# pinellolab/crispr-bean

Measured on AMD Instinct MI355X. Metric: SVI steps/sec, 50k-guide x 20-sample sorting model, higher is better.
Workload: dtype f64; 1 GPU; variant sorting MixtureNormal: 50000 guides x 5 reps x (4 sort bins + bulk), 10000 targets; one SVI step = draw + ELBO + grad + ClippedAdam; per GPU; config=metric, guides=50000, guides_this_rank=50000, n_reps=5, n_condits=5, parallelism=one screen per GPU x1, loss all-reduce every 100 steps, graph_chunk=64

## Files before the change

crispr-bean_amd/csrc/bean_async_v2.hpp:

```cpp
#pragma once

#include "bean_devargs_sgpr.hpp"

#ifndef BEAN_ASYNC_INLINE
#define BEAN_ASYNC_INLINE __forceinline__
#endif
#ifndef BEAN_ASYNC_PRIO
#define BEAN_ASYNC_PRIO 1
#endif
#ifndef BEAN_ASYNC_SLEEP
#define BEAN_ASYNC_SLEEP 8
#endif
#ifndef BEAN_ASYNC_EU
#define BEAN_ASYNC_EU BEAN_WAVE_EU
#endif

namespace bean {

constexpr long kAsyncMinItems = 2800;
constexpr long kAsyncMaxItems = 24000;
__host__ __device__ inline int async_waves_per_simd(long items, long simds = 1024) {
    const double per_simd = (double)items / (double)(simds > 0 ? simds : 1);
    return per_simd <= 5400.0 / 1024.0 ? 2 : (per_simd <= 11000.0 / 1024.0 ? 3 : 4);
}
__host__ __device__ inline bool async_size_in_range(long items, long simds = 1024) {
    const double per_simd = (double)items / (double)(simds > 0 ? simds : 1);
    return per_simd >= (double)kAsyncMinItems / 1024.0 && per_simd <= (double)kAsyncMaxItems / 1024.0;
}
__host__ __device__ inline bool async_finisher_roles(int waves_per_simd, long items, long simds) {
    const double per_wave = (double)items / (double)(waves_per_simd * simds);
    return (waves_per_simd == 2 && per_wave >= 0.95) || (waves_per_simd == 3 && per_wave >= 2.4);
}
constexpr int kAsyncQueueStride = 32;
constexpr int kAsyncStealEvery = 64;
constexpr int kAsyncSpinMax = 1 << 21;

struct AsyncArgs {
    unsigned long long step0, slot0;
    int n_steps;
    int* queue;
    int* done;
    int* abort_flag;
    int n_guide_blocks;
    int fin_split;
    int* fhead;
    int* fring;
    long fring_stride;
    const float* step_sizes;
    unsigned long long* stamps;
};
constexpr int kAsyncStampStep0 = 40, kAsyncStampSteps = 4;
constexpr long kAsyncStampFinOff = 1l << 22;
#ifdef BEAN_ASYNC_STAMP
#define BEAN_ASYNC_T(k)                                                                              \
    if (st_row) {                                                                                    \
        unsigned long long u_;                                                                       \
        asm volatile("s_memrealtime %0\n\ts_waitcnt lgkmcnt(0)" : "=s"(u_)::"memory");               \
        if (lane == 0) st_row[k] = u_;                                                               \
    }
#define BEAN_ASYNC_TF(k)                                                                             \
    if (st_row) {                                                                                    \
        unsigned long long u_;                                                                       \
        asm volatile("s_memrealtime %0\n\ts_waitcnt lgkmcnt(0)" : "=s"(u_)::"memory");               \
        if (lane == 0) st_row[kAsyncStampFinOff + (k)] = u_;                                         \
    }
#define BEAN_ASYNC_ST_ARG , unsigned long long* st_row
#define BEAN_ASYNC_ST_PASS , st_row
#define BEAN_ASYNC_ST_DRAW , (st_row ? st_row + 3 : nullptr)
#else
#define BEAN_ASYNC_T(k)
#define BEAN_ASYNC_TF(k)
#define BEAN_ASYNC_ST_ARG
#define BEAN_ASYNC_ST_PASS
#define BEAN_ASYNC_ST_DRAW
#endif

__global__ __launch_bounds__(64) void k_put_args(DevArgs c, DevArgs* out) {
    const unsigned int* src = (const unsigned int*)&c;
    unsigned int* dst = (unsigned int*)out;
    for (unsigned i = threadIdx.x; i < sizeof(DevArgs) / 4; i += 64) dst[i] = src[i];
}

__global__ __launch_bounds__(256) void k_step_sizes(DevArgs c, unsigned long long step0, int n, float* out) {
    const int i = blockIdx.x * blockDim.x + threadIdx.x;
    if (i < n) out[i] = adam_coef(c, step0 + (unsigned long long)i + 1).step_size;
}

__global__ __launch_bounds__(256) void k_async_head(DevArgs c, AsyncArgs a, DevArgs* args_out, int* ws, int ws_ints,
                                                    float* step_sizes) {
    const long tid = (long)blockIdx.x * 256 + threadIdx.x, nth = (long)gridDim.x * 256;
    for (long i = tid; i < 8 * a.fring_stride; i += nth) a.fring[i] = 0;
    if (blockIdx.x != 0) return;
    for (int i = threadIdx.x; i < ws_ints; i += 256) ws[i] = 0;
    for (int i = threadIdx.x; i < c.n_arrival_ctr; i += 256) c.tile_ctr[i] = 0;
    for (int i = threadIdx.x; i < a.n_steps; i += 256) step_sizes[i] = adam_coef(c, a.step0 + (unsigned long long)i + 1).step_size;
    const unsigned int* src = (const unsigned int*)&c;
    unsigned int* dst = (unsigned int*)args_out;
    for (unsigned i = threadIdx.x; i < sizeof(DevArgs) / 4; i += 256) dst[i] = src[i];
    if (threadIdx.x != 0) return;
    StepCtr last, next;
    last.step = a.step0 + a.n_steps - 1;
    last.slot = a.slot0 + a.n_steps - 1;
    last.step_size = adam_coef(c, last.step + 1).step_size;
    last.pad_ = 0.f;
    next.step = last.step + 1;
    next.slot = last.slot + 1;
    next.step_size = 0.f;
    next.pad_ = 0.f;
    *c.ctrA = last;
    *c.ctrB = next;
}

__device__ __forceinline__ void async_give_up(const DevArgs* cp, const AsyncArgs& a) {
    __hip_atomic_store(a.abort_flag, 1, __ATOMIC_RELAXED, __HIP_MEMORY_SCOPE_AGENT);
    long long* acc = cp->loss_acc;
    for (int i = 0; i < a.n_steps; ++i)
        atomicAdd((unsigned long long*)(acc + ((long)(a.slot0 + i) * kLossSub) * kLossWords) + 2, 1ull);
}

constexpr int kAsyncFinDone = 0, kAsyncFinLeave = 1, kAsyncFinGaveUp = 2;
template <int FAM, bool ACC>
__device__ BEAN_ASYNC_INLINE int async_finish_tile(const DevArgs* cp, unsigned long long step, unsigned long long slot,
                                              float step_size, int tile, int part, const int* wait_slot,
                                              const int* abort_flag BEAN_ASYNC_ST_ARG) {
    if (BEAN_ASYNC_PRIO && !wait_slot) __builtin_amdgcn_s_setprio(3);
    const DevArgs c = dev_args_in_sgprs(cp);
    part = rfl_i(part);
    step = rfl_u64(step);
    slot = rfl_u64(slot);
    step_size = __builtin_bit_cast(float, rfl_i(__builtin_bit_cast(int, step_size)));
    tile = rfl_i(tile);
    int t0, nt;
    {
        const int gf = tile * 64 - c.g_sh > 0 ? tile * 64 - c.g_sh : 0;
        const int gl = tile * 64 + 63 - c.g_sh < c.G ? tile * 64 + 63 - c.g_sh : c.G - 1;
        const int gv = c.g2t[threadIdx.x == 0 ? gf : gl];
        t0 = __builtin_amdgcn_readlane(gv, 0);
        nt = __builtin_amdgcn_readlane(gv, 1) - t0 + 1;
    }
    StepCtr ctr;
    ctr.step = step;
    ctr.slot = slot;
    ctr.step_size = step_size;
    ctr.pad_ = 0.f;
    constexpr bool MIX = FAM == kMixture;
    constexpr int COH = 2;
    extern __shared__ double tabs[];
    const int lane = threadIdx.x, R = c.R, G = c.G, B = c.B;
    const int t1 = t0 + nt - 1;
    int tof0, tof1;
    {
        const int tv = c.toff[lane == 0 ? t0 : t1 + 1];
        tof0 = __builtin_amdgcn_readlane(tv, 0);
        tof1 = __builtin_amdgcn_readlane(tv, 1);
    }
    if (wait_slot) {
        int spins = 0;
        for (;;) {
            int v = 0, ab = 0;
            if (lane == 0) v = __hip_atomic_load(wait_slot, __ATOMIC_RELAXED, __HIP_MEMORY_SCOPE_AGENT);
            if (lane == 1) ab = __hip_atomic_load(abort_flag, __ATOMIC_RELAXED, __HIP_MEMORY_SCOPE_AGENT);
            if (__any(ab != 0)) return kAsyncFinLeave;
            if (__builtin_amdgcn_readfirstlane(v) != 0) break;
            if (++spins > kAsyncSpinMax) return kAsyncFinGaveUp;
            __builtin_amdgcn_s_sleep(BEAN_ASYNC_SLEEP);
        }
        if (BEAN_ASYNC_PRIO) __builtin_amdgcn_s_setprio(3);
    }
    asm volatile("" ::: "memory");
    BEAN_ASYNC_TF(part == 2 ? 6 : 4);
    const unsigned long long s_prep = ctr.step + 1;
    AdamCoef ak;
    ak.step_size = ctr.step_size;
    ak.clip = (float)c.clip;
    const int g_first = tile * 64 - c.g_sh > 0 ? tile * 64 - c.g_sh : 0;
    const int g_last = tile * 64 + 63 - c.g_sh < G ? tile * 64 + 63 - c.g_sh : G - 1;
    const bool left_str = tof0 < g_first;
    const bool right_str = tof1 > g_last + 1;
    long long loss_hi = 0, loss_lo = 0, loss_bad = 0;
    auto loss_term = [&](double v) {
        if (!(fabs(v) < kLossPartMax)) {
            loss_bad = 1;
            return;
        }
        const double hi = rint(v * 1024.0);
        loss_hi += (long long)hi;
        loss_lo += (long long)rint((v - hi * (1.0 / 1024.0)) * 1099511627776.0);
    };
    if (part & 1) {
    int own_left = left_str ? 0 : 1, own_right = right_str ? 0 : 1;
    {
        int* const bp = c.bnd_ctr + (lane == 0 ? (left_str ? tile - 1 : tile) : tile);
        int old = 0;
        if ((lane == 0 && left_str) || (lane == 1 && right_str))
            old = __hip_atomic_fetch_add(bp, 1, __ATOMIC_RELAXED, __HIP_MEMORY_SCOPE_AGENT);
        const int ol = __builtin_amdgcn_readlane(old, 0), orr = __builtin_amdgcn_readlane(old, 1);
        if (left_str && (ol & 1)) own_left = 1;
        if (right_str && (orr & 1)) own_right = 1;
    }
    BEAN_ASYNC_TF(0);
    const int ta = own_left ? t0 : t0 + 1, tb = own_right ? t1 : t1 - 1;
    double* hmu = tabs;
    double* hy = tabs + 64;
    __syncthreads();

    {
        const int j = lane & 3;
        float* const P = j == 0 ? c.p[0] : (j == 1 ? c.p[1] : (j == 2 ? c.p[2] : c.p[3]));
        float* const M = j == 0 ? c.m[0] : (j == 1 ? c.m[1] : (j == 2 ? c.m[2] : c.m[3]));
        float* const V = j == 0 ? c.v[0] : (j == 1 ? c.v[1] : (j == 2 ? c.v[2] : c.v[3]));
        for (int base = ta; base <= tb; base += 16) {
            const int t = base + (lane >> 2);
            const bool act = t <= tb;
            const int tc = act ? t : tb;
            int2 dsc;
            dsc.x = 0;
            dsc.y = 2;
            if (!c.tsum_direct) dsc = c.tdesc[tc];
            const int n = dsc.y * R, ntm = c.tile_targets;
            const long S = c.tsum_direct ? 2 * (long)c.T : (long)c.n_tiles * ntm;
            float pj = coh_ld<COH>(P + tc), mj = coh_ld<COH>(M + tc), vj = coh_ld<COH>(V + tc);
            const float p1 = coh_ld<COH>(c.p[1] + tc), p3 = coh_ld<COH>(c.p[3] + tc);
            const double eps1 = coh_ld<COH>(c.eps_mu + tc), eps2 = coh_ld<COH>(c.eps_sd + tc);
            const double mu = coh_ld<COH>(c.mu_t + tc), y = coh_ld<COH>(c.y_t + tc);
            double am[4] = {0.0, 0.0, 0.0, 0.0}, ay[4] = {0.0, 0.0, 0.0, 0.0};
            const float rR = 1.0f / (float)R;
            for (int i0 = 0; i0 < n; i0 += 32) {
                double xm[2][4], xy[2][4];
#pragma unroll
                for (int mm = 0; mm < 2; ++mm)
#pragma unroll
                    for (int k = 0; k < 4; ++k) {
                        const int i = i0 + 16 * mm + j + 4 * k;
                        xm[mm][k] = 0.0;
                        xy[mm][k] = 0.0;
                        if (act && i < n) {
                            const int part = (int)(((float)i + 0.5f) * rR), rr = i - part * R;
                            const long o = (long)rr * S + (c.tsum_direct ? 2 * (long)tc + part
                                                                         : (part == 0 ? dsc.x : (dsc.x / ntm + part) * ntm));
                            xm[mm][k] = row_ld<true>(c.tsum + o);
                            xy[mm][k] = row_ld<true>(c.tsum + (long)R * S + o);
                        }
                    }
#pragma unroll
                for (int mm = 0; mm < 2; ++mm)
#pragma unroll
                    for (int k = 0; k < 4; ++k) {
                        const int i = i0 + 16 * mm + j + 4 * k;
                        if (act && i < n) {
                            am[k] += xm[mm][k];
                            ay[k] += xy[mm][k];
                        }
                    }
            }
            double gmu = (am[0] + am[2]) + (am[1] + am[3]);
            double gy = (ay[0] + ay[2]) + (ay[1] + ay[3]);
            gmu += __shfl_xor(gmu, 2, 64);
            gy += __shfl_xor(gy, 2, 64);
            gmu += __shfl_xor(gmu, 1, 64);
            gy += __shfl_xor(gy, 1, 64);
            double dlogp_mu, dlogp_dy, lt;
            tgt_prior_terms(c, tc, tgt_sd_prior(c, tc), mu, y, eps1, eps2, p1, p3, dlogp_mu, dlogp_dy, lt);
            if (act && j == 0) loss_term(lt);
            const double Gd = j < 2 ? gmu - dlogp_mu : gy - dlogp_dy;
            const double grad = tgt_grad(j, Gd, j < 2 ? eps1 : eps2, exp((double)pj));
            adam_update(pj, mj, vj, (float)grad, ak);
            if (act) {
                coh_st<COH>(P + t, pj);
                coh_st<COH>(M + t, mj);
                coh_st<COH>(V + t, vj);
            }
            const float2 nrm = normal2_at(c.seed, ((unsigned long long)kSiteTarget << 48) + (unsigned long long)(c.t_off + tc),
                                          s_prep * 4ull);
            const double en = j < 2 ? (double)nrm.x : (double)nrm.y;
            const float p_scale = __shfl_xor(pj, 1, 64);
            const double val = tgt_draw(pj, en, p_scale);
            if (act && (j & 1) == 0) {
                coh_st<COH>((j == 0 ? c.eps_mu : c.eps_sd) + t, en);
                coh_st<COH>((j == 0 ? c.mu_t : c.y_t) + t, val);
                (j == 0 ? hmu : hy)[t - ta] = val;
            }
        }
    }
    __syncthreads();
    BEAN_ASYNC_TF(1);
    {
#pragma clang fp contract(off)
        const int nue = c.ue_idx[2 * B];
        const int nu1 = nue > 0 ? nue : 1, per = 64 / nu1;
        double* const ecdf = tabs + 128;
        double* const epdf = ecdf + 64;
        double* const eupd = epdf + 64;
        for (int base = ta; base <= tb; base += per) {
            const int grp = lane / nu1, ue = lane - grp * nu1;
            const int t = base + grp;
            const bool live = grp < per && t <= tb && nue > 0;
            const int tl = live ? t - ta : 0;
            {
                const double mu = hmu[tl], y = hy[tl];
                const double sigma = c.family == kNormal ? exp(0.5 * y) : exp(y);
                const double inv = 1.0 / sigma;
                const double u = (c.ue_z[live ? ue : 0] - mu) * inv;
                const double pdf = norm_pdf(u);
                if (live) {
                    ecdf[lane] = norm_cdf(u);
                    epdf[lane] = pdf;
                    eupd[lane] = u * pdf;
                }
            }
            __syncthreads();
            const int cnt = (tb - base + 1 < per ? tb - base + 1 : per) * B;
            for (int q = lane; q < cnt; q += 64) {
                const int gq = q / B, b = q - gq * B, tq = base + gq;
                const double y = hy[tq - ta];
                const double sigma = c.family == kNormal ? exp(0.5 * y) : exp(y);
                const double dsig_dy = c.family == kNormal ? 0.5 * sigma : sigma;
                const double inv = 1.0 / sigma;
                const int ih = c.ue_idx[b], il = c.ue_idx[B + b];
                const double ch = ih < 0 ? 1.0 : ecdf[gq * nu1 + ih], cl = il < 0 ? 0.0 : ecdf[gq * nu1 + il];
                const double fh = ih < 0 ? 0.0 : epdf[gq * nu1 + ih], fl = il < 0 ? 0.0 : epdf[gq * nu1 + il];
                const double uh = ih < 0 ? 0.0 : eupd[gq * nu1 + ih], ul = il < 0 ? 0.0 : eupd[gq * nu1 + il];
                const long o = (long)b * c.T + tq;
                coh_st<COH>(c.tabP + o, ch - cl);
                coh_st<COH>(c.tabPmu + o, -(fh - fl) * inv);
                coh_st<COH>(c.tabPy + o, -(uh - ul) * inv * dsig_dy);
            }
            __syncthreads();
        }
    }
    }
    BEAN_ASYNC_TF(2);
    if (MIX && (part & 2)) {
        const int g = tile * 64 + lane - c.g_sh;
        double lg = 0.0;
        if (g >= 0 && g < G) {
            param_guide_mix<true, true, true, COH>(c, g, ak, s_prep, lg);
            loss_term(lg);
        }
    }
    BEAN_ASYNC_TF(3);
    if (part & 1) {
        for (int r0 = 0; r0 < R; r0 += 64) {
            if (r0 + lane < R) {
                const long long* o = c.lpart + 3 * (long)(((tile >> 3) * R + r0 + lane) * 8 + (tile & 7));
                loss_hi += __hip_atomic_load(o, __ATOMIC_RELAXED, __HIP_MEMORY_SCOPE_AGENT);
                loss_lo += __hip_atomic_load(o + 1, __ATOMIC_RELAXED, __HIP_MEMORY_SCOPE_AGENT);
                loss_bad += __hip_atomic_load(o + 2, __ATOMIC_RELAXED, __HIP_MEMORY_SCOPE_AGENT);
            }
        }
    }
    loss_hi = wave_sum_i64(loss_hi);
    loss_lo = wave_sum_i64(loss_lo);
    loss_bad = wave_sum_i64(loss_bad);
    if (lane == 0) {
        long long a = 0, b = 0, d = 0;
        a += loss_hi;
        b += loss_lo;
        d += loss_bad;
        long long* acc = c.loss_acc + ((long)ctr.slot * kLossSub + (tile & (kLossSub - 1))) * kLossWords;
        atomicAdd((unsigned long long*)acc, (unsigned long long)a);
        atomicAdd((unsigned long long*)acc + 1, (unsigned long long)b);
        if (d) atomicAdd((unsigned long long*)acc + 2, (unsigned long long)d);
    }
    return kAsyncFinDone;
}

template <int FAM, bool ACC>
__device__ BEAN_ASYNC_INLINE int2 async_guide_item(const DevArgs& c, W2Prep& pp, bool stage_now, unsigned long long step,
                                              unsigned long long slot, float step_size, int tile,
                                              int r BEAN_ASYNC_ST_ARG) {
    StepCtr ctr;
    ctr.step = rfl_u64(step);
    ctr.slot = rfl_u64(slot);
    ctr.step_size = __builtin_bit_cast(float, rfl_i(__builtin_bit_cast(int, step_size)));
    ctr.pad_ = 0.f;
    const int lane = threadIdx.x, R = c.R;
    const int wg = ((tile >> 3) * R + r) * 8 + (tile & 7);
    int t0, nt;
    double tot;
    guide_wave2_rest<FAM, ACC, 2>(c, ctr, tile, r, wg, pp, stage_now, t0, nt, tot BEAN_ASYNC_ST_DRAW);
    BEAN_ASYNC_T(4);
    if (lane == 0) {
        long long w0 = 0, w1 = 0, w2 = 1;
        if (fabs(tot) < kLossPartMax) {
            const double hi = rint(tot * 1024.0);
            w0 = (long long)hi;
            w1 = (long long)rint((tot - hi * (1.0 / 1024.0)) * 1099511627776.0);
            w2 = 0;
        }
        long long* o = c.lpart + 3 * (long)wg;
        __hip_atomic_store(o, w0, __ATOMIC_RELAXED, __HIP_MEMORY_SCOPE_AGENT);
        __hip_atomic_store(o + 1, w1, __ATOMIC_RELAXED, __HIP_MEMORY_SCOPE_AGENT);
        __hip_atomic_store(o + 2, w2, __ATOMIC_RELAXED, __HIP_MEMORY_SCOPE_AGENT);
    }
    asm volatile("s_waitcnt vmcnt(0)" ::: "memory");
    int last = 0;
    if (lane == 0) {
        const int old = __hip_atomic_fetch_add(c.tile_ctr + tile, 1, __ATOMIC_RELAXED, __HIP_MEMORY_SCOPE_AGENT);
        if (old % R == R - 1) last = 1;
    }
    last = __builtin_amdgcn_readfirstlane(last);
// ... 77 lines not shown
            int w = __hip_atomic_load(pw, __ATOMIC_RELAXED, __HIP_MEMORY_SCOPE_AGENT);
            asm volatile("" ::: "memory");
            const DevArgs c = dev_args_in_sgprs(cp);
            const int tile_u = rfl_i(tile), r_u = rfl_i(r);
            const unsigned long long step = a.step0 + (unsigned long long)s, slot = a.slot0 + (unsigned long long)s;
            W2Prep pp;
            guide_wave2_prepare<FAM, ACC, 2>(c, rfl_u64(step), tile_u, r_u, pp);
            int v = need ? w : s, ab = lane == 4 ? w : 0;
            if (__any(ab != 0)) return;
            bool ready = __all(v >= s);
            const bool fast = ready;
            if (!ready) {
                {
                    const int lane_st = w2_lane_here();
                    guide_wave2_stage_counts<FAM>(c, lane_st, tile_u, r_u, pp);
                    guide_wave2_stage<FAM, 3>(c, lane_st, tile_u, r_u, pp);
                }
                int spins = 0;
                for (;;) {
                    if (++spins > kAsyncSpinMax) {
                        if (lane == 0) async_give_up(cp, a);
                        return;
                    }
                    if (roles && (spins & (kAsyncStealEvery - 1)) == 0) {
                        int e = 0;
                        if (lane == 0) {
                            const int h = __hip_atomic_load(fhead, __ATOMIC_RELAXED, __HIP_MEMORY_SCOPE_AGENT);
                            if (h < total_fin) {
                                const int cand = __hip_atomic_load(fring + h, __ATOMIC_RELAXED, __HIP_MEMORY_SCOPE_AGENT);
                                int expect = h;
                                if (cand != 0 && __hip_atomic_compare_exchange_strong(fhead, &expect, h + 1, __ATOMIC_RELAXED,
                                                                                      __ATOMIC_RELAXED, __HIP_MEMORY_SCOPE_AGENT))
                                    e = h + 1;
                            }
                        }
                        e = __builtin_amdgcn_readfirstlane(e);
                        if (e != 0) {
                            int jt;
                            async_fin_pos(e - 1, nx, a.fin_split, fin_s, jt, fin_part);
                            fin_tile = jt * 8 + x;
                            break;
                        }
                    }
                    __builtin_amdgcn_s_sleep(BEAN_ASYNC_SLEEP);
                    w = __hip_atomic_load(pw, __ATOMIC_RELAXED, __HIP_MEMORY_SCOPE_AGENT);
                    v = need ? w : s;
                    ab = lane == 4 ? w : 0;
                    if (__any(ab != 0)) return;
                    if (__all(v >= s)) {
                        ready = true;
                        break;
                    }
                }
            }
            asm volatile("" ::: "memory");
            BEAN_ASYNC_T(1);
            if (ready) {
                const int2 fin = async_guide_item<FAM, ACC>(c, pp, fast, step, slot, a.step_sizes[s], tile_u, r_u BEAN_ASYNC_ST_PASS);
                item = -1;
                BEAN_ASYNC_T(2);
                if (fin.x >= 0) {
                    if (roles) {
                        if (lane == 0) {
                            int* const w = fring + (long)(s * nx + jt) * (a.fin_split ? 2 : 1);
                            __hip_atomic_store(w, s + 1, __ATOMIC_RELAXED, __HIP_MEMORY_SCOPE_AGENT);
                            if (a.fin_split) __hip_atomic_store(w + 1, s + 1, __ATOMIC_RELAXED, __HIP_MEMORY_SCOPE_AGENT);
                        }
                    } else {
                        fin_s = s;
                        fin_tile = tile;
                        fin_part = 3;
                    }
                }
            }
        }
        if (fin_s >= 0) {
#ifdef BEAN_ASYNC_STAMP
            st_row = nullptr;
            if (a.stamps && fin_s >= kAsyncStampStep0 && fin_s < kAsyncStampStep0 + kAsyncStampSteps)
                st_row = a.stamps + ((long)(fin_s - kAsyncStampStep0) * ((long)((n_tiles + 7) / 8 * 8) * R) + (long)fin_tile * R) * 8;
#endif
            const unsigned long long step = a.step0 + (unsigned long long)fin_s, slot = a.slot0 + (unsigned long long)fin_s;
            const int left = async_finish_tile<FAM, ACC>(cp, step, slot, a.step_sizes[fin_s], fin_tile, fin_part, fin_wait,
                                                         a.abort_flag BEAN_ASYNC_ST_PASS);
            if (BEAN_ASYNC_PRIO) __builtin_amdgcn_s_setprio(0);
            if (left != kAsyncFinDone) {
                if (left == kAsyncFinGaveUp && lane == 0) async_give_up(cp, a);
                return;
            }
            asm volatile("s_waitcnt vmcnt(0)" ::: "memory");
            if (lane == 0) {
                if (fin_part & 1) __hip_atomic_store(a.done + 2 * fin_tile, fin_s + 1, __ATOMIC_RELAXED, __HIP_MEMORY_SCOPE_AGENT);
                if (fin_part & 2) __hip_atomic_store(a.done + 2 * fin_tile + 1, fin_s + 1, __ATOMIC_RELAXED, __HIP_MEMORY_SCOPE_AGENT);
            }
            BEAN_ASYNC_TF(fin_part == 2 ? 7 : 5);
        }
        __syncthreads();
    }
}

}
```

crispr-bean_amd/csrc/bean_hip.hip:

```cpp
#include <hip/hip_runtime.h>
#include <hip/hip_ext.h>
#include <stdio.h>
#include <stdlib.h>
#include <string.h>
#include <dlfcn.h>
#include <rccl/rccl.h>

#include <string>
#include <type_traits>
#include <vector>

#include "../../include/bean_hip.h"
#include "bean_kernels.hpp"
#include "bean_predictive.hpp"
#include "bean_importance.hpp"
#include "bean_importance_marg.hpp"
#include "bean_grid.hpp"

using namespace bean;

static thread_local std::string g_err;
static int fail(const std::string& msg) {
    g_err = msg;
    return -1;
}
#define HIP_OK(expr)                                                                 \
    do {                                                                             \
        hipError_t e_ = (expr);                                                      \
        if (e_ != hipSuccess)                                                        \
            return fail(std::string(#expr) + ": " + hipGetErrorString(e_));          \
    } while (0)

struct ArgSet {
    DevArgs* dev = nullptr;
    std::vector<DevArgs> host;
    std::vector<uint64_t> seeds;
    bool dirty = true;
    std::vector<hipGraphExec_t> ladder;
};

struct bean_hip_ctx {
    bean_hip_shape shape = {};
    DevArgs d = {};
    void* slot_ptr[BEAN_BUF_COUNT] = {};
    uint64_t slot_bytes[BEAN_BUF_COUNT] = {};
    void* workspace = nullptr;
    uint64_t workspace_bytes = 0;
    uint64_t loss_capacity = 0;
    bool prepared = false;
    bool fused_guide = true;
    bool wave_guide = false;
    bool wave2 = false;
    bool surv_wave = false;
    bool fused_step = false;
    std::vector<hipGraphExec_t> graphs_fused;
    long long* loss_acc = nullptr;
    int* tile_targets_dev = nullptr;
    double* tsum_buf = nullptr;
    int2* tdesc_buf = nullptr;
    int* live_slots = nullptr;
    bool tiling_wave = false;
    bool tiling_wide = false;
    int tiling_rep_w = 0;
    bool tiling_rep = false;
    bool alleles_fresh = false;
    bool allele_blocks = true;
    bool resume_head_fresh = false;
    double* gsum_ws = nullptr;
    double* sq_ws = nullptr;
    double* cov_sum_ws = nullptr;
    std::vector<hipGraphExec_t> graphs;
    unsigned long long graph_seed = 0;
    bool profile = false;
    bool profile_param = false;
    std::vector<hipEvent_t> ev;
    bool tile_svi = false;
    bool tile_ready = false;
    int* tile_tab = nullptr;
    int n_tiles = 0, tile_ntm = 0, tile_gbm = 0, tile_blocks = 0;
    float* step_sizes = nullptr;
    DevArgs* dargs_dev = nullptr;
    uint64_t step_sizes_cap = 0;
    std::vector<uint64_t> ev_steps;
    ncclComm_t comm = nullptr;
    int comm_world = 0;
    std::vector<hipGraphExec_t> graphs_xchg;
    std::vector<hipGraphExec_t> graphs_resume;
    bool resume_ok = false;
    uint64_t sharded_steps = 0;
    uint64_t resume_next = 0, resume_seed = 0;
    void* resume_stream = nullptr;
    bool async_step = false;
    bool dirgrad_tab = true;
    int* async_ws = nullptr;
    int async_blocks = 0;
    int async_fin_blocks = 0;
    size_t async_ws_ints = 0;
    unsigned long long* async_stamps = nullptr;
    size_t async_stamp_words = 0;
    int n_members = 1;
    bool bound_any = false;
    char* member_ws = nullptr;
    size_t member_ws_stride = 0;
    size_t tsum_stride = 0;
    ArgSet members;
    bool members_set = false;
    const uint8_t* member_rg = nullptr;
    const double* member_smask = nullptr;
    const float* member_x = nullptr;
    const float* member_xbc = nullptr;
    int n_particles = 1;
    bool particles_set = false;
    float* particle_grad = nullptr;
    double* particle_loss = nullptr;
    ArgSet particles;
};

extern "C" const char* bean_hip_version(void) {
    return BEAN_AMAX <= 8 ? "bean_hip 0.1.0 (gfx950)"
                          : (BEAN_AMAX <= 16 ? "bean_hip 0.1.0 (gfx950, 16 alleles per guide / 16 conditions)"
                                             : "bean_hip 0.1.0 (gfx950, 32 alleles per guide / 16 conditions)");
}
extern "C" const char* bean_hip_last_error(void) { return g_err.c_str(); }

static bool is_survival(const bean_hip_shape& s) { return s.selection == BEAN_SELECTION_SURVIVAL; }
static bool is_tiling(const bean_hip_shape& s) { return s.family == BEAN_FAMILY_MULTI_MIXTURE; }
static bool is_surv_normal(const bean_hip_shape& s) {
    return s.selection == BEAN_SELECTION_SURVIVAL && s.family == BEAN_FAMILY_NORMAL;
}
static bool is_mixture(const bean_hip_shape& s) {
    return s.family == BEAN_FAMILY_MIXTURE_NORMAL || s.family == BEAN_FAMILY_MULTI_MIXTURE;
}

template <typename F>
static auto with_family_acc(const DevArgs& d, F&& f) {
    if (d.family == kMixture) {
        if (d.flags & kAcc) return f(std::integral_constant<int, kMixture>{}, std::true_type{});
        return f(std::integral_constant<int, kMixture>{}, std::false_type{});
    }
    return f(std::integral_constant<int, kNormal>{}, std::false_type{});
}
template <typename F>
static auto with_acc_surv(const DevArgs& d, F&& f) {
    if (d.survival) {
        if (d.flags & kAcc) return f(std::true_type{}, std::true_type{});
        return f(std::false_type{}, std::true_type{});
    }
    if (d.flags & kAcc) return f(std::true_type{}, std::false_type{});
    return f(std::false_type{}, std::false_type{});
}

static uint64_t expected_bytes(const bean_hip_shape& s, int slot) {
    const uint64_t R = s.n_reps, B = s.n_condits, G = s.n_guides, T = s.n_targets;
    const uint64_t A = s.n_max_alleles, C = s.n_ctrl;
    auto param_elems = [&](int i) -> uint64_t {
        switch (i) {
            case 0: case 1: return T;
            case 2: case 3: return is_survival(s) ? 0 : T;
            case 7: return ((is_survival(s) && s.family == BEAN_FAMILY_MIXTURE_NORMAL) || is_surv_normal(s)) ? G : 0;
            case 4: return is_mixture(s) ? G * A : 0;
            case 5: case 6:
                if (s.n_sample_covariates > 0) return (uint64_t)s.n_sample_covariates;
                return (is_mixture(s) && (s.flags & BEAN_FLAG_SCALE_BY_ACC) && (s.flags & BEAN_FLAG_FIT_NOISE)) ? G : 0;
        }
        return 0;
    };
    if (slot >= BEAN_BUF_P_MU_LOC && slot < BEAN_BUF_P_MU_LOC + 8) return 4 * param_elems(slot - BEAN_BUF_P_MU_LOC);
    if (slot >= BEAN_BUF_G_MU_LOC && slot < BEAN_BUF_G_MU_LOC + 8) return 4 * param_elems(slot - BEAN_BUF_G_MU_LOC);
    if (slot >= BEAN_BUF_M_MU_LOC && slot < BEAN_BUF_M_MU_LOC + 8) return 4 * param_elems(slot - BEAN_BUF_M_MU_LOC);
    if (slot >= BEAN_BUF_V_MU_LOC && slot < BEAN_BUF_V_MU_LOC + 8) return 4 * param_elems(slot - BEAN_BUF_V_MU_LOC);
    switch (slot) {
        case BEAN_BUF_X: return 4 * R * B * G;
        case BEAN_BUF_X_BC: return (s.flags & BEAN_FLAG_USE_BCMATCH) ? 4 * R * B * G : 0;
        case BEAN_BUF_ALLELE_CTRL: return is_mixture(s) ? 4 * R * C * G * A : 0;
        case BEAN_BUF_REPGUIDE: return R * G;
        case BEAN_BUF_SIZE_FACTOR: return 8 * R * B;
        case BEAN_BUF_SIZE_FACTOR_BC: return (s.flags & BEAN_FLAG_USE_BCMATCH) ? 8 * R * B : 0;
        case BEAN_BUF_SAMPLE_MASK: return 8 * R * B;
        case BEAN_BUF_A0: return 8 * G;
// ... 293 lines not shown
        if (!c->fused_guide || !c->wave2 || !c->surv_wave || !c->tiling_wave ||
            (stp && (!strcmp(stp, "fused") || !strcmp(stp, "tile")))) {
            delete c;
            return fail("bean_hip_create: BEAN_HIP_GUIDE / _SURVIVAL / _TILING=block / _STEP select A/B reference kernels, "
                        "which this build does not contain (build with -DBEAN_AB_KERNELS: libbean_hip_ab.so)");
        }
#endif
    }
    {
        const char* am = getenv("BEAN_HIP_ALLELE");
        c->allele_blocks = !(am && !strcmp(am, "split"));
    }
    DevArgs& d = c->d;
    d.R = s->n_reps; d.B = s->n_condits; d.G = s->n_guides; d.T = s->n_targets;
    d.A = s->n_max_alleles; d.C = s->n_ctrl; d.E = s->n_edits;
    d.family = s->family; d.flags = s->flags; d.mask_thres = s->mask_thres;
    d.wide_targets = (!is_tiling(*s) && (s->n_targets < 64 || s->max_target_len > 256)) ? 1 : 0;
    d.lpt = kLanesPerTarget;
    if (is_tiling(*s)) {
        if ((int64_t)s->n_a2e_nnz <= 16 * (int64_t)s->n_targets) d.lpt = kLanesPerTargetNarrow;
    } else if (is_survival(*s)) {
        d.lpt = kLanesPerTargetNarrow;
    }
    d.g_off = s->guide_offset; d.t_off = s->target_offset;
    d.G_tot = s->n_guides_total > 0 ? s->n_guides_total : s->n_guides;
    d.sd_prior_scale = s->sd_prior_scale; d.lr0 = s->initial_lr; d.log_lrd = log(s->lrd);
    d.clip = s->clip_norm;
    d.survival = is_survival(*s) ? 1 : 0;
    d.neg_loc = s->negctrl_loc; d.neg_scale = s->negctrl_scale;

    const uint64_t G = d.G;
    const bool surv_mix = is_survival(*s) && s->family == BEAN_FAMILY_MIXTURE_NORMAL;
    const bool surv_norm = is_surv_normal(*s);
    d.surv_q0lik = surv_norm ? 1 : 0;
    d.not_loss_owner = (s->flags & BEAN_FLAG_NOT_LOSS_OWNER) ? 1 : 0;
    d.q0_blocks = (surv_mix || surv_norm) ? 1 : 0;
    d.q0_blk0 = surv_mix ? (int)((G + kParamBlock - 1) / kParamBlock) : 0;
    d.n_gamma_blocks = (int)((G + kParamBlock - 1) / kParamBlock);
    const bool split_ok = !is_survival(*s) && !is_tiling(*s);
    c->wave_guide = c->wave_guide && split_ok;
    c->wave2 = c->wave2 && c->wave_guide;
    if (s->n_sample_covariates > 0 && !c->wave2) {
        delete c;
        return fail("bean_hip_create: sample covariates need the default guide kernel (k_guide_wave2)");
    }
    d.n_cov = s->n_sample_covariates;
    d.g_sh = c->wave2 ? s->guide_offset % 64 : 0;
    d.n_tiles = (int)((d.g_sh + G + 63) / 64);
    {
        const int seg = s->max_target_len < 1 ? 64 : (s->max_target_len > 64 ? 64 : s->max_target_len);
        d.seg_steps = 0;
        while ((1 << d.seg_steps) < seg) ++d.seg_steps;
    }
    c->surv_wave =c->surv_wave && is_survival(*s) && !is_tiling(*s);
    d.rows_v2 = (c->wave2 || c->surv_wave) ? 1 : 0;

    c->tiling_wide = is_tiling(*s) && s->n_max_alleles > kAMax;
    c->tiling_wave = c->tiling_wave && is_tiling(*s) && !c->tiling_wide;
    {
        const char* tmode = getenv("BEAN_HIP_TILING");
        c->tiling_rep = c->tiling_wave && s->n_reps <= kTilingRepMaxR && !(tmode && !strcmp(tmode, "wave"));
        if (c->tiling_rep) c->tiling_wave = false;
        const int w_env = getenv("BEAN_HIP_TILING_W") ? atoi(getenv("BEAN_HIP_TILING_W")) : 0;
        long n_simd = 0;
        {
            int dev = 0, n_cu = 0;
            if (hipGetDevice(&dev) == hipSuccess &&
                hipDeviceGetAttribute(&n_cu, hipDeviceAttributeMultiprocessorCount, dev) == hipSuccess)
                n_simd = 4l * n_cu;
            else
                (void)hipGetLastError();
        }
        c->tiling_rep_w = (w_env == 1 || w_env == 2 || w_env == 4)
                              ? w_env
                              : tiling_rep_waves(s->n_reps, s->n_condits, (s->flags & BEAN_FLAG_SCALE_BY_ACC) != 0,
                                                 (long)s->n_guides, n_simd);
        if (s->n_condits > 16) c->tiling_rep_w = 1;
    }
    d.wide_alleles = c->tiling_wide ? 1 : 0;
    {
        const char* dt = getenv("BEAN_HIP_DIRGRAD_TAB");
        c->dirgrad_tab = !(dt && !strcmp(dt, "0"));
    }
    d.trow_summed = (c->tiling_wave || c->tiling_rep) ? 1 : 0;
    {
        const char* tc = getenv("BEAN_HIP_TOT_CONST");
        d.tot_const = ((c->wave2 || c->surv_wave || c->tiling_wave || c->tiling_rep || c->tiling_wide) && !(tc && !strcmp(tc, "0"))) ? 1 : 0;
    }
#ifdef BEAN_AB_KERNELS
    {
        const char* sm = getenv("BEAN_HIP_STEP");
        c->fused_step = c->wave2 && !d.wide_targets && s->max_target_len <= 64 && s->n_sample_covariates == 0 &&
                        (s->family == BEAN_FAMILY_MIXTURE_NORMAL || s->family == BEAN_FAMILY_NORMAL) &&
                        (sm && !strcmp(sm, "fused"));
    }
    {
        const char* sm = getenv("BEAN_HIP_STEP");
        const int gb = s->n_reps <= 64 ? kTileThreads / s->n_reps : 0;
        c->tile_svi = c->wave2 && !d.wide_targets && s->n_sample_covariates == 0 && !c->fused_step &&
                      (s->family == BEAN_FAMILY_MIXTURE_NORMAL || s->family == BEAN_FAMILY_NORMAL) &&
                      gb >= 1 && s->max_target_len <= gb && (sm && !strcmp(sm, "tile"));
    }
#endif
    {
        const char* sm = getenv("BEAN_HIP_STEP");
        const long items = (long)d.n_tiles * s->n_reps;
        int dev_ = 0, n_cu_ = 256;
        if (hipGetDevice(&dev_) != hipSuccess || hipDeviceGetAttribute(&n_cu_, hipDeviceAttributeMultiprocessorCount, dev_) != hipSuccess)
            n_cu_ = 256;
        (void)hipGetLastError();
        const bool on = sm ? !strcmp(sm, "async") : async_size_in_range(items, 4l * n_cu_);
        c->async_step = on && c->wave2 && !d.wide_targets && s->max_target_len <= 64 && s->n_sample_covariates == 0 &&
                        !c->fused_step && !c->tile_svi &&
                        (s->family == BEAN_FAMILY_MIXTURE_NORMAL || s->family == BEAN_FAMILY_NORMAL) && !is_survival(*s);
    }
    const uint64_t tiles8 = ((uint64_t)d.n_tiles + 7) / 8 * 8;
    d.n_arrival_ctr = c->wave2 ? (int)(2 * (tiles8 + 2)) : (is_tiling(*s) ? 2 * kAlleleCtrLines * 16 : 0);
    d.n_lpart = (c->wave2 || c->surv_wave) ? (int)(tiles8 * (uint64_t)d.R) : 0;
    d.tile_targets = 64;
    uint64_t n_measured = 0;
    workspace_regions(c, d, [&](auto&, uint64_t n) { n_measured += n; });
    c->workspace_bytes = n_measured * 8;
    hipError_t e = hipMalloc(&c->workspace, c->workspace_bytes);
    if (e != hipSuccess) {
        delete c;
        return fail(std::string("hipMalloc workspace: ") + hipGetErrorString(e));
    }
    e = hipMemset(c->workspace, 0, c->workspace_bytes);
    if (e != hipSuccess) {
        (void)hipFree(c->workspace);
        delete c;
        return fail(std::string("hipMemset workspace: ") + hipGetErrorString(e));
    }
    double* w = (double*)c->workspace;
    workspace_regions(c, d, [&](auto& p, uint64_t n) {
        p = (std::remove_reference_t<decltype(p)>)w;
        w += n;
    }, &c->tile_targets_dev);
    if ((uint64_t)(w - (double*)c->workspace) != n_measured) {
        const std::string msg = "bean_hip_create: the workspace regions take " + std::to_string(w - (double*)c->workspace) +
                                " doubles, " + std::to_string(n_measured) + " were measured";
        (void)hipFree(c->workspace);
        delete c;
        return fail(msg);
    }
    c->gsum_ws = d.gsum;
    c->sq_ws = d.sq;
    c->cov_sum_ws = d.cov_sum;
    *out = c;
    return 0;
}

extern "C" int bean_hip_comm_destroy(bean_hip_ctx* c);
extern "C" int bean_hip_destroy(bean_hip_ctx* c) {
    if (!c) return 0;
    drop_graph(c);
    (void)bean_hip_comm_destroy(c);
    for (hipEvent_t e : c->ev) (void)hipEventDestroy(e);
    if (c->workspace) (void)hipFree(c->workspace);
    if (c->tile_tab) (void)hipFree(c->tile_tab);
    if (c->live_slots) (void)hipFree(c->live_slots);
    if (c->tsum_buf) (void)hipFree(c->tsum_buf);
    if (c->tdesc_buf) (void)hipFree(c->tdesc_buf);
    if (c->step_sizes) (void)hipFree(c->step_sizes);
    if (c->dargs_dev) (void)hipFree(c->dargs_dev);
    if (c->async_ws) (void)hipFree(c->async_ws);
// ... 808 lines not shown
    const DevArgs& d = c->d;
    const size_t lds = guide_wave2_lds(d.B, d.tile_targets);
    if (c->async_blocks == 0) {
        int per_cu = 0, dev = 0, n_cu = 0;
        if (lds > 65536)
            HIP_OK(hipFuncSetAttribute((const void*)k_svi_async<FAM, ACC>, hipFuncAttributeMaxDynamicSharedMemorySize, (int)lds));
        HIP_OK(hipOccupancyMaxActiveBlocksPerMultiprocessor(&per_cu, k_svi_async<FAM, ACC>, 64, lds));
        HIP_OK(hipGetDevice(&dev));
        HIP_OK(hipDeviceGetAttribute(&n_cu, hipDeviceAttributeMultiprocessorCount, dev));
        if (per_cu < 1) return fail("k_svi_async does not fit on a compute unit (LDS " + std::to_string(lds) + " bytes)");
        int k = async_waves_per_simd((long)d.n_tiles * d.R, 4l * n_cu);
        if (k > per_cu / 4) k = per_cu / 4;
        c->async_blocks = k >= 1 ? k * 4 * n_cu : per_cu * n_cu / 8 * 8;
        c->async_fin_blocks = (k >= 1 && k + 1 <= per_cu / 4 && async_finisher_roles(k, (long)d.n_tiles * d.R, 4l * n_cu)) ? 4 * n_cu : 0;
        if (const char* e = getenv("BEAN_HIP_ASYNC_BLOCKS")) {
            const int v = atoi(e) / 8 * 8;
            if (v >= 8) c->async_blocks = v;
        }
        if (const char* e = getenv("BEAN_HIP_ASYNC_FIN")) {
            const int v = atoi(e);
            c->async_fin_blocks = v < 0 ? -1 : v / 8 * 8;
        }
        if (getenv("BEAN_HIP_VERBOSE"))
            fprintf(stderr, "k_svi_async: %d tiles x %d replicates per step, LDS %zu B, %d workgroups per CU x %d CUs -> grid %d\n",
                    d.n_tiles, d.R, lds, per_cu, n_cu, c->async_blocks);
    }
    const long items = (long)((d.n_tiles + 7) / 8 * 8) * d.R;
    int blocks = c->async_blocks;
    if ((long)blocks > items) blocks = (int)((items + 7) / 8 * 8);
    AsyncArgs a = a_in;
    int fin_blocks = 0;
    a.fin_split = (double)d.n_tiles * d.R / (double)(c->async_blocks > 0 ? c->async_blocks : 1) < 2.15 ? 1 : 0;
    if (const char* e = getenv("BEAN_HIP_ASYNC_SPLIT")) a.fin_split = atoi(e) != 0;
    if (c->async_fin_blocks != 0 && a.fring_stride > 0 && d.n_tiles <= 8 * 65535) {
        fin_blocks = c->async_fin_blocks < 0 ? 0 : c->async_fin_blocks;
        const int tiles8 = (d.n_tiles + 7) / 8 * 8;
        if (fin_blocks > tiles8) fin_blocks = tiles8;
        a.n_guide_blocks = blocks;
        blocks += fin_blocks;
    } else {
        a.n_guide_blocks = 0;
    }
    const bool prof = prof_guide(c);
    launch_timed(c, prof, k_svi_async<FAM, ACC>, dim3(blocks), dim3(64), lds, stream, (const DevArgs*)c->dargs_dev, d.R,
                 d.n_tiles, a);
    if (prof) c->ev_steps.push_back((uint64_t)a.n_steps);
    if (roles_out) *roles_out = a.n_guide_blocks;
    return 0;
}

static int launch_svi_async(bean_hip_ctx* c, hipStream_t stream, uint64_t step0, uint64_t slot0, uint64_t n_steps) {
    const DevArgs& d = c->d;
    if (n_steps > c->step_sizes_cap) {
        if (c->step_sizes) (void)hipFree(c->step_sizes);
        c->step_sizes = nullptr;
        c->step_sizes_cap = 0;
        const uint64_t cap = n_steps < 256 ? 256 : n_steps;
        HIP_OK(hipMalloc((void**)&c->step_sizes, cap * sizeof(float)));
        c->step_sizes_cap = cap;
    }
    const size_t ws_ints = (size_t)17 * kAsyncQueueStride + (size_t)2 * d.n_tiles;
    const size_t fring_stride = n_steps < 8000 ? (size_t)2 * ((d.n_tiles + 7) / 8) * n_steps : 0;
    const size_t need_ints = ws_ints + 8 * fring_stride;
    if (need_ints > c->async_ws_ints) {
        if (c->async_ws) (void)hipFree(c->async_ws);
        c->async_ws = nullptr;
        c->async_ws_ints = 0;
        HIP_OK(hipMalloc((void**)&c->async_ws, need_ints * sizeof(int)));
        c->async_ws_ints = need_ints;
    }
    if (!c->dargs_dev) HIP_OK(hipMalloc((void**)&c->dargs_dev, sizeof(DevArgs)));
    AsyncArgs a;
    a.step0 = step0;
    a.slot0 = slot0;
    a.n_steps = (int)n_steps;
    a.queue = c->async_ws;
    a.abort_flag = c->async_ws + 8 * kAsyncQueueStride;
    a.fhead = c->async_ws + 9 * kAsyncQueueStride;
    a.done = c->async_ws + 17 * kAsyncQueueStride;
    a.fring = c->async_ws + ws_ints;
    a.fring_stride = (long)fring_stride;
    a.n_guide_blocks = 0;
    a.fin_split = 0;
    a.step_sizes = c->step_sizes;
    a.stamps = nullptr;
    {
        unsigned hb = (unsigned)((8 * fring_stride + 256 * 64 - 1) / (256 * 64));
        if (hb < 1) hb = 1;
        if (hb > 128) hb = 128;
        hipLaunchKernelGGL(k_async_head, dim3(hb), dim3(256), 0, stream, d, a, c->dargs_dev, c->async_ws, (int)ws_ints, c->step_sizes);
    }
#ifdef BEAN_ASYNC_STAMP
    {
        static unsigned long long* g_stamps = nullptr;
        const size_t words = (size_t)2 * kAsyncStampFinOff;
        if ((size_t)kAsyncStampSteps * ((d.n_tiles + 7) / 8 * 8) * d.R * 8 > (size_t)kAsyncStampFinOff)
            return fail("BEAN_ASYNC_STAMP: screen too large for the stamp buffer");
        if (!g_stamps) HIP_OK(hipMalloc((void**)&g_stamps, words * 8));
        HIP_OK(hipMemsetAsync(g_stamps, 0, words * 8, stream));
        a.stamps = g_stamps;
        c->async_stamps = g_stamps;
        c->async_stamp_words = words;
    }
#endif
    return with_family_acc(d, [&](auto fam, auto acc) { return launch_svi_async_t<fam(), acc()>(c, stream, a, nullptr); });
}

extern "C" int bean_hip_svi_run(bean_hip_ctx* c, uint64_t seed, uint64_t first_step, uint64_t n_steps,
                                int32_t graph_chunk, void* stream_) {
    const int go = begin_steps(c, "bean_hip_svi_run", first_step, n_steps);
    if (go <= 0) return go;
    hipStream_t stream = (hipStream_t)stream_;
    drop_graph_on_seed_change(c, seed);
    c->d.seed = seed;
    c->resume_ok = false;
    const DevArgs& dd = c->d;
    const bool tile = c->tile_svi && c->tile_ready && !c->profile_param && !per_step_noise(dd) && !dumps_pi(dd);
    const bool use_graph = graph_chunk > 0 && stream != nullptr && !c->profile && !tile;
    const bool fused = c->fused_step && !c->profile_param && !per_step_noise(dd);
    auto pairs_n = [&](uint64_t n) {
        enqueue_pairs(c, stream, n);
        return 0;
    };
    if (use_graph) {
        const int kmax = top_rung(graph_chunk, 1, 10);
        std::vector<hipGraphExec_t>& ladder = fused ? c->graphs_fused : c->graphs;
        const int n_rungs = fused ? (kmax > 0 ? kmax : 1) : kmax + 1;
        if ((int)ladder.size() != n_rungs) {
            drop_graph(c);
            auto fused_n = [&](uint64_t n) {
                enqueue_fused(c, stream, n);
                return 0;
            };
            const int rc = fused ? build_ladder(c, ladder, stream, n_rungs, 2, c->alleles_fresh, fused_n)
                                 : build_ladder(c, ladder, stream, n_rungs, 1, c->alleles_fresh, pairs_n);
            if (rc) {
                drop_graph(c);
                return -1;
            }
            c->graph_seed = seed;
        }
    }
    first_draw(c, stream, first_step, n_steps);
    if (tile) {
#ifdef BEAN_AB_KERNELS
        if (launch_svi_tile(c, stream, first_step, n_steps)) return -1;
#endif
    } else if (async_candidate(c, n_steps) && stream != nullptr) {
        if (launch_svi_async(c, stream, first_step, first_step, n_steps)) return -1;
    } else if (fused) {
        uint64_t left = n_steps;
        if (use_graph) {
            for (int k = (int)c->graphs_fused.size() - 1; k >= 0; --k)
                while (left >= (2ull << k)) {
                    HIP_OK(hipGraphLaunch(c->graphs_fused[k], stream));
                    left -= 2ull << k;
                }
        }
        enqueue_fused(c, stream, left);
    } else {
        launch_guide(c, stream);
        if (use_graph) {
            if (replay_pairs(c, c->graphs, stream, n_steps - 1, pairs_n)) return -1;
        } else {
            enqueue_pairs(c, stream, n_steps - 1);
        }
// ... 1164 lines not shown
```

Measured before the change: 22800 steps/s.

## Prefetch finisher target state and RNG draws into LDS before waiting on slot

Finisher tiles that must wait on a slot now do independent work before spinning. They stage the ue_z/ue_idx tables and precompute the next-step normal draws and target descriptors into shared memory. If neighbouring tiles' done counters show the state is already final, they also load the Adam state and compute the prior terms early, then reuse these values after the wait. This hides global-load and RNG latency behind the spin wait, at the cost of extra LDS use, more register pressure, and a correctness dependence on the done-counter gating.

```diff
diff --git a/crispr-bean_amd/csrc/bean_async_v2.hpp b/crispr-bean_amd/csrc/bean_async_v2.hpp
--- a/crispr-bean_amd/csrc/bean_async_v2.hpp
+++ b/crispr-bean_amd/csrc/bean_async_v2.hpp
@@ -43,6 +43,7 @@
     int* abort_flag;
     int n_guide_blocks;
     int fin_split;
+    int early;
     int* fhead;
     int* fring;
     long fring_stride;
@@ -122,8 +123,18 @@
 template <int FAM, bool ACC>
 __device__ BEAN_ASYNC_INLINE int async_finish_tile(const DevArgs* cp, unsigned long long step, unsigned long long slot,
                                               float step_size, int tile, int part, const int* wait_slot,
-                                              const int* abort_flag BEAN_ASYNC_ST_ARG) {
+                                              const int* abort_flag, const int* done, int s_local, int n_tiles,
+                                              int early BEAN_ASYNC_ST_ARG) {
     if (BEAN_ASYNC_PRIO && !wait_slot) __builtin_amdgcn_s_setprio(3);
+    const bool try_early = wait_slot != nullptr && early != 0 && (part & 1) != 0;
+    int gate_w = 0;
+    if (try_early && early == 1) {
+        const int ln = w2_lane_here();
+        const int q = ln == 1 ? tile - 1 : (ln == 2 ? tile + 1 : tile);
+        const int qc = q < 0 ? 0 : (q >= n_tiles ? n_tiles - 1 : q);
+        gate_w = __hip_atomic_load(done + 2 * qc, __ATOMIC_RELAXED, __HIP_MEMORY_SCOPE_AGENT);
+        asm volatile("" ::: "memory");
+    }
     const DevArgs c = dev_args_in_sgprs(cp);
     part = rfl_i(part);
     step = rfl_u64(step);
@@ -146,13 +157,77 @@
     constexpr bool MIX = FAM == kMixture;
     constexpr int COH = 2;
     extern __shared__ double tabs[];
-    const int lane = threadIdx.x, R = c.R, G = c.G, B = c.B;
+    const int lane = w2_lane_here(), R = c.R, G = c.G, B = c.B;
     const int t1 = t0 + nt - 1;
     int tof0, tof1;
     {
         const int tv = c.toff[lane == 0 ? t0 : t1 + 1];
         tof0 = __builtin_amdgcn_readlane(tv, 0);
         tof1 = __builtin_amdgcn_readlane(tv, 1);
+    }
+    const int g_first = tile * 64 - c.g_sh > 0 ? tile * 64 - c.g_sh : 0;
+    const int g_last = tile * 64 + 63 - c.g_sh < G ? tile * 64 + 63 - c.g_sh : G - 1;
+    const bool left_str = tof0 < g_first;
+    const bool right_str = tof1 > g_last + 1;
+    constexpr int kEarlyN = 68, kEarlySlots = 128, kEarlyUe = 608;
+    double* const es_eps = tabs + kEarlySlots;
+    double* const es_dlp = es_eps + kEarlyN;
+    double* const es_lt = es_dlp + kEarlyN;
+    double* const es_exp = es_lt + kEarlyN;
+    float* const es_p = (float*)(es_exp + kEarlyN);
+    int2* const es_dsc = (int2*)(es_exp + kEarlyN + 2 * kEarlyN);
+    double* const ue_zs = tabs + kEarlyUe;
+    int* const ue_is = (int*)(ue_zs + 2 * B);
+    bool pre_static = false, pre_state = false;
+    if (try_early && guide_wave2_lds(B, c.tile_targets) >= (size_t)(kEarlyUe + 2 * B) * sizeof(double) + (size_t)(2 * B + 1) * sizeof(int)) {
+        pre_static = true;
+        const int ln = w2_lane_here();
+        const int j = ln & 3;
+        if (early == 1) {
+            const bool need = ln == 0 || (ln == 1 && left_str && tile > 0) || (ln == 2 && right_str && tile + 1 < n_tiles);
+            pre_state = __all(!need || gate_w >= s_local);
+        }
+        asm volatile("" ::: "memory");
+        for (int i = ln; i < 2 * B; i += 64) ue_zs[i] = c.ue_z[i];
+        for (int i = ln; i <= 2 * B; i += 64) ue_is[i] = c.ue_idx[i];
+        auto prep = [&](int sl, int tp) {
+            float pj = 0.f, mj = 0.f, vj = 0.f, p1 = 0.f, p3 = 0.f;
+            double eps1 = 0.0, eps2 = 0.0, mu = 0.0, y = 0.0;
+            if (pre_state) {
+                const float* const P = j == 0 ? c.p[0] : (j == 1 ? c.p[1] : (j == 2 ? c.p[2] : c.p[3]));
+                const float* const M = j == 0 ? c.m[0] : (j == 1 ? c.m[1] : (j == 2 ? c.m[2] : c.m[3]));
+                const float* const V = j == 0 ? c.v[0] : (j == 1 ? c.v[1] : (j == 2 ? c.v[2] : c.v[3]));
+                pj = coh_ld<COH>(P + tp), mj = coh_ld<COH>(M + tp), vj = coh_ld<COH>(V + tp);
+                p1 = coh_ld<COH>(c.p[1] + tp), p3 = coh_ld<COH>(c.p[3] + tp);
+                eps1 = coh_ld<COH>(c.eps_mu + tp), eps2 = coh_ld<COH>(c.eps_sd + tp);
+                mu = coh_ld<COH>(c.mu_t + tp), y = coh_ld<COH>(c.y_t + tp);
+            }
+            int2 dsc;
+            dsc.x = 0;
+            dsc.y = 2;
+            if (!c.tsum_direct) dsc = c.tdesc[tp];
+            const float2 nrm = normal2_at(c.seed, ((unsigned long long)kSiteTarget << 48) + (unsigned long long)(c.t_off + tp),
+                                          (step + 1) * 4ull);
+            es_p[3 * kEarlyN + sl] = j < 2 ? nrm.x : nrm.y;
+            es_dsc[sl] = dsc;
+            if (pre_state) {
+                double dlogp_mu, dlogp_dy, lt;
+                tgt_prior_terms(c, tp, tgt_sd_prior(c, tp), mu, y, eps1, eps2, p1, p3, dlogp_mu, dlogp_dy, lt);
+                es_eps[sl] = j < 2 ? eps1 : eps2;
+                es_dlp[sl] = j < 2 ? dlogp_mu : dlogp_dy;
+                es_lt[sl] = lt;
+                es_exp[sl] = exp((double)pj);
+                es_p[sl] = pj;
+                es_p[kEarlyN + sl] = mj;
+                es_p[2 * kEarlyN + sl] = vj;
+            }
+        };
+        const int rounds = left_str && t0 + 16 <= t1 ? 2 : 1;
+#pragma clang loop unroll(disable)
+        for (int rd = 0; rd < rounds; ++rd) {
+            const int k = rd * 16 + (ln >> 2);
+            if (rd == 0 || ln < 4) prep(k * 4 + j, t0 + k < t1 ? t0 + k : t1);
+        }
     }
     if (wait_slot) {
         int spins = 0;
@@ -173,10 +248,6 @@
     AdamCoef ak;
     ak.step_size = ctr.step_size;
     ak.clip = (float)c.clip;
-    const int g_first = tile * 64 - c.g_sh > 0 ? tile * 64 - c.g_sh : 0;
-    const int g_last = tile * 64 + 63 - c.g_sh < G ? tile * 64 + 63 - c.g_sh : G - 1;
-    const bool left_str = tof0 < g_first;
-    const bool right_str = tof1 > g_last + 1;
     long long loss_hi = 0, loss_lo = 0, loss_bad = 0;
     auto loss_term = [&](double v) {
         if (!(fabs(v) < kLossPartMax)) {
@@ -210,19 +281,27 @@
         float* const M = j == 0 ? c.m[0] : (j == 1 ? c.m[1] : (j == 2 ? c.m[2] : c.m[3]));
         float* const V = j == 0 ? c.v[0] : (j == 1 ? c.v[1] : (j == 2 ? c.v[2] : c.v[3]));
         for (int base = ta; base <= tb; base += 16) {
+            const bool pre = pre_static && base == ta, pre_s = pre && pre_state;
             const int t = base + (lane >> 2);
             const bool act = t <= tb;
             const int tc = act ? t : tb;
+            const int es = (tc - t0) * 4 + j;
             int2 dsc;
             dsc.x = 0;
             dsc.y = 2;
-            if (!c.tsum_direct) dsc = c.tdesc[tc];
+            if (pre) dsc = es_dsc[es];
+            else if (!c.tsum_direct) dsc = c.tdesc[tc];
             const int n = dsc.y * R, ntm = c.tile_targets;
             const long S = c.tsum_direct ? 2 * (long)c.T : (long)c.n_tiles * ntm;
-            float pj = coh_ld<COH>(P + tc), mj = coh_ld<COH>(M + tc), vj = coh_ld<COH>(V + tc);
-            const float p1 = coh_ld<COH>(c.p[1] + tc), p3 = coh_ld<COH>(c.p[3] + tc);
-            const double eps1 = coh_ld<COH>(c.eps_mu + tc), eps2 = coh_ld<COH>(c.eps_sd + tc);
-            const double mu = coh_ld<COH>(c.mu_t + tc), y = coh_ld<COH>(c.y_t + tc);
+            float pj = 0.f, mj = 0.f, vj = 0.f, p1 = 0.f, p3 = 0.f;
+            double eps1 = 0.0, eps2 = 0.0, mu = 0.0, y = 0.0;
+            double epsj = 0.0, dlogp = 0.0, lt = 0.0, spj = 0.0;
+            if (!pre_s) {
+                pj = coh_ld<COH>(P + tc), mj = coh_ld<COH>(M + tc), vj = coh_ld<COH>(V + tc);
+                p1 = coh_ld<COH>(c.p[1] + tc), p3 = coh_ld<COH>(c.p[3] + tc);
+                eps1 = coh_ld<COH>(c.eps_mu + tc), eps2 = coh_ld<COH>(c.eps_sd + tc);
+                mu = coh_ld<COH>(c.mu_t + tc), y = coh_ld<COH>(c.y_t + tc);
+            }
             double am[4] = {0.0, 0.0, 0.0, 0.0}, ay[4] = {0.0, 0.0, 0.0, 0.0};
             const float rR = 1.0f / (float)R;
             for (int i0 = 0; i0 < n; i0 += 32) {
@@ -259,20 +338,33 @@
             gy += __shfl_xor(gy, 2, 64);
             gmu += __shfl_xor(gmu, 1, 64);
             gy += __shfl_xor(gy, 1, 64);
-            double dlogp_mu, dlogp_dy, lt;
-            tgt_prior_terms(c, tc, tgt_sd_prior(c, tc), mu, y, eps1, eps2, p1, p3, dlogp_mu, dlogp_dy, lt);
+            if (pre_s) {
+                pj = es_p[es], mj = es_p[kEarlyN + es], vj = es_p[2 * kEarlyN + es];
+                epsj = es_eps[es], dlogp = es_dlp[es], lt = es_lt[es], spj = es_exp[es];
+            } else {
+                double dlogp_mu, dlogp_dy;
+                tgt_prior_terms(c, tc, tgt_sd_prior(c, tc), mu, y, eps1, eps2, p1, p3, dlogp_mu, dlogp_dy, lt);
+                epsj = j < 2 ? eps1 : eps2;
+                dlogp = j < 2 ? dlogp_mu : dlogp_dy;
+                spj = exp((double)pj);
+            }
             if (act && j == 0) loss_term(lt);
-            const double Gd = j < 2 ? gmu - dlogp_mu : gy - dlogp_dy;
-            const double grad = tgt_grad(j, Gd, j < 2 ? eps1 : eps2, exp((double)pj));
+            const double Gd = (j < 2 ? gmu : gy) - dlogp;
+            const double grad = tgt_grad(j, Gd, epsj, spj);
             adam_update(pj, mj, vj, (float)grad, ak);
             if (act) {
                 coh_st<COH>(P + t, pj);
                 coh_st<COH>(M + t, mj);
                 coh_st<COH>(V + t, vj);
             }
-            const float2 nrm = normal2_at(c.seed, ((unsigned long long)kSiteTarget << 48) + (unsigned long long)(c.t_off + tc),
-                                          s_prep * 4ull);
-            const double en = j < 2 ? (double)nrm.x : (double)nrm.y;
+            double en;
+            if (pre) {
+                en = (double)es_p[3 * kEarlyN + es];
+            } else {
+                const float2 nrm = normal2_at(c.seed, ((unsigned long long)kSiteTarget << 48) + (unsigned long long)(c.t_off + tc),
+                                              s_prep * 4ull);
+                en = j < 2 ? (double)nrm.x : (double)nrm.y;
+            }
             const float p_scale = __shfl_xor(pj, 1, 64);
             const double val = tgt_draw(pj, en, p_scale);
             if (act && (j & 1) == 0) {
@@ -286,7 +378,10 @@
     BEAN_ASYNC_TF(1);
     {
 #pragma clang fp contract(off)
-        const int nue = c.ue_idx[2 * B];
+        const bool staged = pre_static;
+        int nue;
+        if (staged) nue = __builtin_amdgcn_readfirstlane(ue_is[2 * B]);
+        else nue = c.ue_idx[2 * B];
         const int nu1 = nue > 0 ? nue : 1, per = 64 / nu1;
         double* const ecdf = tabs + 128;
         double* const epdf = ecdf + 64;
@@ -297,10 +392,13 @@
             const bool live = grp < per && t <= tb && nue > 0;
             const int tl = live ? t - ta : 0;
             {
+                double z;
+                if (staged) z = ue_zs[live ? ue : 0];
+                else z = c.ue_z[live ? ue : 0];
                 const double mu = hmu[tl], y = hy[tl];
                 const double sigma = c.family == kNormal ? exp(0.5 * y) : exp(y);
                 const double inv = 1.0 / sigma;
-                const double u = (c.ue_z[live ? ue : 0] - mu) * inv;
+                const double u = (z - mu) * inv;
                 const double pdf = norm_pdf(u);
                 if (live) {
                     ecdf[lane] = norm_cdf(u);
@@ -312,11 +410,13 @@
             const int cnt = (tb - base + 1 < per ? tb - base + 1 : per) * B;
             for (int q = lane; q < cnt; q += 64) {
                 const int gq = q / B, b = q - gq * B, tq = base + gq;
+                int ih, il;
+                if (staged) ih = ue_is[b], il = ue_is[B + b];
+                else ih = c.ue_idx[b], il = c.ue_idx[B + b];
                 const double y = hy[tq - ta];
                 const double sigma = c.family == kNormal ? exp(0.5 * y) : exp(y);
                 const double dsig_dy = c.family == kNormal ? 0.5 * sigma : sigma;
                 const double inv = 1.0 / sigma;
-                const int ih = c.ue_idx[b], il = c.ue_idx[B + b];
                 const double ch = ih < 0 ? 1.0 : ecdf[gq * nu1 + ih], cl = il < 0 ? 0.0 : ecdf[gq * nu1 + il];
                 const double fh = ih < 0 ? 0.0 : epdf[gq * nu1 + ih], fl = il < 0 ? 0.0 : epdf[gq * nu1 + il];
                 const double uh = ih < 0 ? 0.0 : eupd[gq * nu1 + ih], ul = il < 0 ? 0.0 : eupd[gq * nu1 + il];
@@ -560,7 +660,7 @@
 #endif
             const unsigned long long step = a.step0 + (unsigned long long)fin_s, slot = a.slot0 + (unsigned long long)fin_s;
             const int left = async_finish_tile<FAM, ACC>(cp, step, slot, a.step_sizes[fin_s], fin_tile, fin_part, fin_wait,
-                                                         a.abort_flag BEAN_ASYNC_ST_PASS);
+                                                         a.abort_flag, a.done, fin_s, n_tiles, a.early BEAN_ASYNC_ST_PASS);
             if (BEAN_ASYNC_PRIO) __builtin_amdgcn_s_setprio(0);
             if (left != kAsyncFinDone) {
                 if (left == kAsyncFinGaveUp && lane == 0) async_give_up(cp, a);
diff --git a/crispr-bean_amd/csrc/bean_hip.hip b/crispr-bean_amd/csrc/bean_hip.hip
--- a/crispr-bean_amd/csrc/bean_hip.hip
+++ b/crispr-bean_amd/csrc/bean_hip.hip
@@ -95,6 +95,7 @@
     int* async_ws = nullptr;
     int async_blocks = 0;
     int async_fin_blocks = 0;
+    int async_early = 1;
     size_t async_ws_ints = 0;
     unsigned long long* async_stamps = nullptr;
     size_t async_stamp_words = 0;
@@ -554,6 +555,10 @@
         const char* dt = getenv("BEAN_HIP_DIRGRAD_TAB");
         c->dirgrad_tab = !(dt && !strcmp(dt, "0"));
     }
+    {
+        const char* ae = getenv("BEAN_HIP_ASYNC_EARLY");
+        c->async_early = (ae && !strcmp(ae, "0")) ? 0 : ((ae && !strcmp(ae, "2")) ? 2 : 1);
+    }
     d.trow_summed = (c->tiling_wave || c->tiling_rep) ? 1 : 0;
     {
         const char* tc = getenv("BEAN_HIP_TOT_CONST");
@@ -1528,6 +1533,7 @@
     a.fring_stride = (long)fring_stride;
     a.n_guide_blocks = 0;
     a.fin_split = 0;
+    a.early = c->async_early;
     a.step_sizes = c->step_sizes;
     a.stamps = nullptr;
     {
```

New measurement: 23100 steps/s, median of 6. 1.3% higher.
